# pasensio97/SDslam

Hardware: AMD Instinct MI355X
Metric: tracked frames/sec (ORB+ImageAlign+PnP) at 640x480, 1000 kp (higher is better)
Workload: dtype u8; 1 GPU; BASELINE configs[3] at the configs[1] pyramid: 640x480, 8-level x1.2, 1000 kp; ORB extract + ImageAlign (levels 4,3,2) + SearchByProjection + PnP RANSAC (maxIts 200; iterations actually run: tracking.mean_pnp_iterations with --full); pose_solver=pnp, pyramid=8x1.2, unique_scenes=64, inputs=resident in HBM, pose_records=packed on the device every step (single GPU: no collective)

## Files before the change

sdslam_amd/csrc/orb.hip:

```cpp
#include <hip/hip_runtime.h>

#include <algorithm>
#include <cstring>
#include <mutex>
#include <string>
#include <vector>

#include "introselect.h"
#include "introselect_wave.h"
#include "orb_plan.h"
#include "sd_common.h"
#include "sd_sincosf.h"

namespace sd {

static thread_local std::string g_err;
void set_error(const std::string& msg) { g_err = msg; }

#ifndef SD_XCD_REMAP
#define SD_XCD_REMAP 1
#endif
__device__ __forceinline__ void xcd_frame_block(unsigned& frame, unsigned& blk) {
#if SD_XCD_REMAP
  const unsigned nx = gridDim.x, total = nx * gridDim.y;
// ... 365 lines not shown
  for (int k = 0; k < 16; k++) {
    int m9 = min(min(m4[k], m4[(k + 4) & 15]), d[(k + 8) & 15]);
    int M9 = max(max(M4[k], M4[(k + 4) & 15]), d[(k + 8) & 15]);
    a = max(a, m9);
    b = min(b, M9);
  }
  return max(a, -b) - 1;
}

typedef unsigned short fu16;
__device__ __forceinline__ fu16 fmin16(fu16 a, fu16 b) { return a < b ? a : b; }
__device__ __forceinline__ fu16 fmax16(fu16 a, fu16 b) { return a > b ? a : b; }

typedef _Float16 fh2 __attribute__((ext_vector_type(2)));
typedef unsigned short fu2 __attribute__((ext_vector_type(2)));
__device__ __forceinline__ fh2 hmax3(fh2 a, fh2 b, fh2 c) { return __builtin_elementwise_maximum(__builtin_elementwise_maximum(a, b), c); }
__device__ __forceinline__ fh2 hmin3(fh2 a, fh2 b, fh2 c) { return __builtin_elementwise_minimum(__builtin_elementwise_minimum(a, b), c); }
__device__ __forceinline__ fh2 ring_pair(const uint8_t* __restrict__ ca, const uint8_t* __restrict__ cb, int o) {
  const fu2 r = {ca[o], cb[o]};
  return __builtin_bit_cast(fh2, r);
}
__device__ __forceinline__ void fast_ring_score2(const uint8_t* __restrict__ ca, const uint8_t* __restrict__ cb, int tp, int& sa, int& sb) {
  fh2 p[16];
  const int va = ca[0], vb = cb[0];
  p[0] = ring_pair(ca, cb, 3 * tp); p[1] = ring_pair(ca, cb, 3 * tp + 1); p[2] = ring_pair(ca, cb, 2 * tp + 2); p[3] = ring_pair(ca, cb, tp + 3);
  p[4] = ring_pair(ca, cb, 3); p[5] = ring_pair(ca, cb, -tp + 3); p[6] = ring_pair(ca, cb, -2 * tp + 2); p[7] = ring_pair(ca, cb, -3 * tp + 1);
  p[8] = ring_pair(ca, cb, -3 * tp); p[9] = ring_pair(ca, cb, -3 * tp - 1); p[10] = ring_pair(ca, cb, -2 * tp - 2); p[11] = ring_pair(ca, cb, -tp - 3);
  p[12] = ring_pair(ca, cb, -3); p[13] = ring_pair(ca, cb, tp - 3); p[14] = ring_pair(ca, cb, 2 * tp - 2); p[15] = ring_pair(ca, cb, 3 * tp - 1);
  fh2 x3[16], n3[16];
#pragma unroll
  for (int k = 0; k < 16; k++) {
    x3[k] = hmax3(p[k], p[(k + 1) & 15], p[(k + 2) & 15]);
    n3[k] = hmin3(p[k], p[(k + 1) & 15], p[(k + 2) & 15]);
  }
  fh2 x9[16], n9[16];
#pragma unroll
  for (int k = 0; k < 16; k++) {
    x9[k] = hmax3(x3[k], x3[(k + 3) & 15], x3[(k + 6) & 15]);
    n9[k] = hmin3(n3[k], n3[(k + 3) & 15], n3[(k + 6) & 15]);
  }
  fh2 A = hmin3(x9[0], x9[1], x9[2]), B = hmax3(n9[0], n9[1], n9[2]);
#pragma unroll
  for (int k = 3; k < 15; k += 2) {
    A = hmin3(A, x9[k], x9[k + 1]);
    B = hmax3(B, n9[k], n9[k + 1]);
  }
  A = __builtin_elementwise_minimum(A, x9[15]);
  B = __builtin_elementwise_maximum(B, n9[15]);
  const fu2 Au = __builtin_bit_cast(fu2, A), Bu = __builtin_bit_cast(fu2, B);
  sa = max(va - (int)Au.x, (int)Bu.x - va) - 1;
  sb = max(vb - (int)Au.y, (int)Bu.y - vb) - 1;
}

#ifdef SD_PNP_PROF
#define FPROF_FRAMES 256
#define FPROF_CELLS 192
__device__ unsigned long long g_fast_prof_wg[(size_t)FPROF_FRAMES * FPROF_CELLS * 8];
#define FPROF_DECL                                   \
  __shared__ unsigned long long s_fprof[8];          \
  if (threadIdx.x < 8) s_fprof[threadIdx.x] = 0;     \
  long long _pt = clock64()
#define FPROF(i)                                                                 \
  do {                                                                           \
    long long _n = clock64();                                                    \
    if (threadIdx.x == 0) s_fprof[i] += (unsigned long long)(_n - _pt);          \
    _pt = _n;                                                                    \
  } while (0)
#define FPROF_FLUSH                                                                                                   \
  do {                                                                                                                \
    if (threadIdx.x == 0 && frame < FPROF_FRAMES && cell < FPROF_CELLS)                                          \
      for (int _i = 0; _i < 8; _i++) g_fast_prof_wg[((size_t)frame * FPROF_CELLS + cell) * 8 + _i] = s_fprof[_i]; \
  } while (0)
#else
#define FPROF_DECL
#define FPROF(i)
#define FPROF_FLUSH
#endif

extern "C" __device__ __attribute__((const)) int __ockl_wfred_add_i32(int);

#ifndef FAST_STAGE_DEPTH
#define FAST_STAGE_DEPTH 12
#endif

struct FastSrc {
  uint32_t off[SD_MAX_LEVELS];
  int pstride[SD_MAX_LEVELS];
};

__global__ __launch_bounds__(256, 8) void k_fast_cells(const CellGeom* __restrict__ cells, const uint8_t* __restrict__ img0,
                                                    size_t frame_stride, const FastSrc src, int edge, uint32_t* __restrict__ cand,
                                                    uint32_t cand_per_frame, int32_t* __restrict__ cell_count, int ncells_total,
                                                    int cell0, int th) {
  extern __shared__ __attribute__((aligned(16))) uint8_t smem[];
  __shared__ int wcnt[4];
  unsigned uframe, ucell;
  xcd_frame_block(uframe, ucell);
  const int cell = (int)ucell + cell0;
  const CellGeom C = cells[cell];
  const int frame = (int)uframe;
  const int tid = threadIdx.x, lane = tid & 63;
  const int wave = __builtin_amdgcn_readfirstlane(tid >> 6);
  if (C.zw <= 0 || C.zh <= 0) {
    if (tid == 0) cell_count[(size_t)frame * ncells_total + cell] = 0;
    return;
  }
  const uint8_t* img = img0 + (size_t)frame * frame_stride + src.off[C.level];
  const int pstride = src.pstride[C.level];
  uint32_t* out = cand + (size_t)frame * cand_per_frame + C.cand_off;
  const int zw = C.zw, zh = C.zh, S = C.strip_rows;
  const int xs = C.zx0 - 3 + edge;
  const int xa = xs & ~3, sh = xs - xa;
  const int TPW = (sh + zw + 6 + 3) >> 2;
  const int TP = TPW * 4;
  const int SP = (zw + 2 + 3) & ~3;
  const int RPW = (S + 2 + 3) >> 2;
  const int QCAP = RPW * zw;
  uint8_t* tile = smem;
  uint8_t* sc = smem + (size_t)TP * (S + 2 + 6);
  uint16_t* queue = (uint16_t*)(sc + (size_t)SP * (S + 2 + 2)) + (size_t)wave * QCAP;
  const uint32_t qbase = (uint32_t)__builtin_amdgcn_readfirstlane((int)((size_t)TP * (S + 2 + 6) + (size_t)SP * (S + 2 + 2) + (size_t)wave * QCAP * 2));
  const unsigned magic = 0xFFFFFFFFu / (unsigned)zw + 1u;
  const unsigned magic_tpw = 0xFFFFFFFFu / (unsigned)TPW + 1u;
  const unsigned long long lt = lanemask_lt();
  int total = 0;
  FPROF_DECL;

  for (int r0 = 0; r0 < zh; r0 += S) {
    const int r1 = min(r0 + S, zh);
    const int sr0 = max(r0 - 1, 0), sr1 = min(r1 + 1, zh);
    const int nsr = sr1 - sr0;
    const int npr = nsr + 6;
    {
      const uint8_t* g = img + (size_t)(C.zy0 + sr0 - 3 + edge) * pstride + xa;
      const int ndw = __mul24(TPW, npr);
      int t0 = tid;
      asm volatile("" : "+v"(t0));
      for (int i0 = t0; i0 < ndw; i0 += 256 * FAST_STAGE_DEPTH) {
        uint32_t v[FAST_STAGE_DEPTH];
#pragma unroll
        for (int j = 0; j < FAST_STAGE_DEPTH; j++) {
          const int i = i0 + 256 * j;
          const int row = (int)__umulhi((unsigned)i, magic_tpw), wc = i - __mul24(row, TPW);
          v[j] = i < ndw ? *(const uint32_t*)(g + (uint32_t)(__mul24(row, pstride) + wc * 4)) : 0u;
        }
#pragma unroll
        for (int j = 0; j < FAST_STAGE_DEPTH; j++) {
          const int i = i0 + 256 * j;
          if (i < ndw) ((uint32_t*)tile)[i] = v[j];
        }
      }
      FPROF(7);
      const int nsc = ((nsr + 2) * SP) >> 2;
      for (int i = tid; i < nsc; i += 256) ((uint32_t*)sc)[i] = 0;
    }
    __syncthreads();
    FPROF(0);
    const int rpw = (nsr + 3) >> 2;
    const int y_lo = min(wave * rpw, nsr), y_hi = min(y_lo + rpw, nsr);
    int qn = 0;
    {
      const int i_lo = __mul24(y_lo, zw), i_hi = __mul24(y_hi, zw);
      const int pad = TP - zw;
      const uint8_t* tile0 = tile + 3 * TP + 3 + sh;
#ifdef FAST_SKIP_A
      for (int i0 = i_hi; i0 < i_hi; i0 += 64) {
#else
      for (int i0 = i_lo; i0 < i_hi; i0 += 64) {
#endif
        const int i = min(i0 + lane, i_hi - 1);
        const int y = (int)__umulhi((unsigned)i, magic);
        const uint8_t* c = tile0 + (i + __mul24(y, pad));
        const fu16 v = c[0], p0 = c[3 * TP], p4 = c[3], p8 = c[-3 * TP], p12 = c[-3];
        const fu16 D = fmax16(fmin16(p0, p8), fmin16(p4, p12));
        const fu16 Bt = fmin16(fmax16(p0, p8), fmax16(p4, p12));
        const short da = (short)(v - D), db = (short)(Bt - v);
        bool pass = (da > db ? da : db) > (short)th;
        if (i_hi - i0 < 64) pass = pass && (i0 + lane < i_hi);
        const unsigned long long m = __builtin_amdgcn_ballot_w64(pass);
        const int rank = (int)__builtin_amdgcn_mbcnt_hi((unsigned)(m >> 32), __builtin_amdgcn_mbcnt_lo((unsigned)m, 0u));
        if (pass) *(uint16_t*)(smem + (qbase + 2u * (uint32_t)(qn + rank))) = (uint16_t)i;
        qn += __popcll(m);
      }
    }
    FPROF(1);
#ifdef FAST_SKIP_B
    qn = 0;
#endif
    int cn = 0;
    for (int e0 = 0; e0 < qn; e0 += 128) {
      const int ea = e0 + lane, eb = ea + 64;
      bool corner_a = false, corner_b = false;
      unsigned qa = 0, qb = 0;
      if (ea < qn) {
        const bool has_b = eb < qn;
        qa = queue[ea];
        qb = has_b ? queue[eb] : qa;
        const int y_a = (int)__umulhi(qa, magic), x_a = (int)qa - __mul24(y_a, zw);
        const int y_b = (int)__umulhi(qb, magic), x_b = (int)qb - __mul24(y_b, zw);
        int sa, sb;
        fast_ring_score2(tile + __mul24(y_a + 3, TP) + x_a + 3 + sh, tile + __mul24(y_b + 3, TP) + x_b + 3 + sh, TP, sa, sb);
        corner_a = sa >= th;
        corner_b = has_b && sb >= th;
        if (corner_a && sa > 0) sc[__mul24(y_a + 1, SP) + x_a + 1] = (uint8_t)sa;
        if (corner_b && sb > 0) sc[__mul24(y_b + 1, SP) + x_b + 1] = (uint8_t)sb;
      }
      const unsigned long long ma = __builtin_amdgcn_ballot_w64(corner_a);
      if (corner_a) queue[cn + __popcll(ma & lt)] = (uint16_t)qa;
      cn += __popcll(ma);
      const unsigned long long mb = __builtin_amdgcn_ballot_w64(corner_b);
      if (corner_b) queue[cn + __popcll(mb & lt)] = (uint16_t)qb;
      cn += __popcll(mb);
    }
    qn = cn;
#ifdef FAST_SKIP_C
    qn = 0;
#endif
    FPROF(2);
    FPROF(3);
    __syncthreads();
    FPROF(4);
    {
      unsigned long long bits = 0;
      int cnt = 0;
      const int nj = (qn + 63) >> 6;
      for (int j = 0; j < nj; j++) {
        const int e = j * 64 + lane;
        bool keep = false;
        if (e < qn) {
          const unsigned q = queue[e];
          const int y = (int)__umulhi(q, magic), x = (int)q - __mul24(y, zw);
          const int yz = sr0 + y;
          const uint8_t* p = sc + __mul24(y + 1, SP) + x + 1;
          const int s = p[0];
          const int n0 = p[-1], n1 = p[1], n2 = p[-SP - 1], n3 = p[-SP], n4 = p[-SP + 1], n5 = p[SP - 1], n6 = p[SP], n7 = p[SP + 1];
          const int nm = max(max(max(n0, n1), n2), max(max(max(n3, n4), n5), max(n6, n7)));
          keep = (s > 0) & (s > nm) & (yz >= r0) & (yz < r1);
        }
        const unsigned long long m = __builtin_amdgcn_ballot_w64(keep);
        cnt += __popcll(m);
        bits |= (unsigned long long)keep << j;
      }
      if (lane == 0) wcnt[wave] = cnt;
      __syncthreads();
      int base = total;
      for (int w = 0; w < wave; w++) base += wcnt[w];
      const int strip_total = wcnt[0] + wcnt[1] + wcnt[2] + wcnt[3];
      for (int j = 0; j < nj; j++) {
        const bool keep = (bits >> j) & 1ull;
        const unsigned long long m = __builtin_amdgcn_ballot_w64(keep);
        if (keep) {
          const unsigned q = queue[j * 64 + lane];
          const int y = (int)__umulhi(q, magic), x = (int)q - __mul24(y, zw);
          const int s = sc[__mul24(y + 1, SP) + x + 1];
          const unsigned pos = (unsigned)(base + __popcll(m & lt));
          if (pos < C.cap)
            out[pos] = ((uint32_t)s << 24) | ((uint32_t)(C.zy0 + sr0 + y) << 12) | (uint32_t)(C.zx0 + x);
        }
        base += __popcll(m);
      }
      total += strip_total;
    }
    FPROF(5);
    __syncthreads();
    FPROF(6);
  }
  if (tid == 0) cell_count[(size_t)frame * ncells_total + cell] = min(total, (int)C.cap);
  FPROF_FLUSH;
}

#define SEL_WAVES 8
#define SEL_LIST_CAP 1536
#define SEL_MAX_CELLS 512
typedef __attribute__((address_space(3))) uint32_t lds_u32;

__global__ __launch_bounds__(64) void k_select_quota(const OrbPlan* __restrict__ P, const CellGeom* __restrict__ cells,
                                                     const int32_t* __restrict__ cell_count, int32_t* __restrict__ cell_keep,
                                                     int32_t* __restrict__ cell_off, int32_t* __restrict__ lvl_m) {
  extern __shared__ __attribute__((aligned(16))) int s_q[];
  const int frame = blockIdx.x, lane = threadIdx.x, nc = P->ncells;
  int* s_total = s_q;
  int* s_flag = s_q + nc;
  int* s_retain = s_q + 2 * nc;
  int* s_offv = s_q + 3 * nc;
  const int32_t* cc = cell_count + (size_t)frame * nc;
  for (int c = lane; c < nc; c += 64) {
    s_total[c] = cc[c];
    s_flag[c] = cells[c].evaluated;
  }
  sdsel::wave_fence();
  if (lane < P->nlevels) {
    const LevelGeom& L = P->lv[lane];
    int M = 0;
    if (L.ncells > 0 && L.quota > 0) {
      const int nC = L.ncells, c0 = L.cell0, nfc = L.nfeaturesCell;
      int nNoMore = 0, nToDistribute = 0;
      for (int c = c0; c < c0 + nC; c++) {
        const int nKeys = s_total[c];
        if (!s_flag[c]) {
          s_retain[c] = 0;
          s_flag[c] = 0;
          continue;
        }
        if (nKeys > nfc) {
          s_retain[c] = nfc;
          s_flag[c] = 0;
        } else {
          s_retain[c] = nKeys;
          nToDistribute += nfc - nKeys;
          s_flag[c] = 1;
          nNoMore++;
        }
      }
      while (nToDistribute > 0 && nNoMore < nC) {
        const int nNew = nfc + (int)ceilf((float)nToDistribute / (float)(nC - nNoMore));
        nToDistribute = 0;
        for (int c = c0; c < c0 + nC; c++) {
          if (!s_flag[c]) {
            if (s_total[c] > nNew) {
              s_retain[c] = nNew;
            } else {
              s_retain[c] = s_total[c];
              nToDistribute += nNew - s_total[c];
              s_flag[c] = 1;
              nNoMore++;
            }
          }
        }
      }
      for (int c = c0; c < c0 + nC; c++) {
        const int k = min(s_total[c], s_retain[c]);
        s_retain[c] = k;
        s_offv[c] = M;
        M += k;
      }
    } else {
      for (int c = L.cell0; c < L.cell0 + max(L.ncells, 0); c++) { s_retain[c] = 0; s_offv[c] = 0; }
// ... 455 lines not shown

static int build_geometry(sd_orb* h, const HostPlan& hp) {
  const size_t B = h->max_batch;
  const size_t slack = 4096;
  SD_HIP_CHECK(hipMalloc(&h->d_cells, std::max<size_t>(hp.cells.size(), 1) * sizeof(CellGeom)));
  SD_HIP_CHECK(hipMalloc(&h->d_tiles, std::max<size_t>(hp.blur_tiles.size(), 1) * sizeof(BlurTile)));
  SD_HIP_CHECK(hipMalloc(&h->d_coef, std::max<size_t>(hp.coef.size(), 1) * sizeof(int32_t)));
  for (int i = 0; i < h->nsets; i++) {
    SD_HIP_CHECK(hipMalloc(&h->pyr_set[i], hp.plan.pyr_frame_bytes * B + slack));
    SD_HIP_CHECK(hipMemsetAsync(h->pyr_set[i], 0, hp.plan.pyr_frame_bytes * B + slack, h->stream));
  }
  select_set(h, 0);
  SD_HIP_CHECK(hipMalloc(&h->d_blur, hp.plan.pyr_frame_bytes * B + slack));
  SD_HIP_CHECK(hipMalloc(&h->d_cand, std::max<size_t>(hp.plan.cand_per_frame, 1) * B * 4));
  SD_HIP_CHECK(hipMalloc(&h->d_scratch, std::max<size_t>(hp.plan.cand_per_frame, 1) * B * 4));
  SD_HIP_CHECK(hipMalloc(&h->d_cell_count, std::max<size_t>(hp.plan.ncells, 1) * B * 4));
  SD_HIP_CHECK(hipMalloc(&h->d_sel, std::max<size_t>(hp.plan.nsel, 1) * B * 4));
  SD_HIP_CHECK(hipMalloc(&h->d_sel_count, (size_t)h->nlevels * B * 4));
  SD_HIP_CHECK(hipMalloc(&h->d_cell_keep, std::max<size_t>(hp.plan.ncells, 1) * B * 4));
  SD_HIP_CHECK(hipMalloc(&h->d_cell_off, std::max<size_t>(hp.plan.ncells, 1) * B * 4));
  SD_HIP_CHECK(hipMalloc(&h->d_lvl_m, (size_t)h->nlevels * B * 4));
  SD_HIP_CHECK(hipMemsetAsync(h->d_blur, 0, hp.plan.pyr_frame_bytes * B + slack, h->stream));
  if (!hp.cells.empty())
    SD_HIP_CHECK(hipMemcpyAsync(h->d_cells, hp.cells.data(), hp.cells.size() * sizeof(CellGeom), hipMemcpyHostToDevice, h->stream));
  if (!hp.blur_tiles.empty())
    SD_HIP_CHECK(hipMemcpyAsync(h->d_tiles, hp.blur_tiles.data(), hp.blur_tiles.size() * sizeof(BlurTile), hipMemcpyHostToDevice, h->stream));
  if (!hp.coef.empty())
    SD_HIP_CHECK(hipMemcpyAsync(h->d_coef, hp.coef.data(), hp.coef.size() * sizeof(int32_t), hipMemcpyHostToDevice, h->stream));
  SD_HIP_CHECK(hipMemcpyAsync(h->d_plan, &hp.plan, sizeof(OrbPlan), hipMemcpyHostToDevice, h->stream));
  SD_HIP_CHECK(hipStreamSynchronize(h->stream));
  return SD_OK;
}

static int ensure_geometry(sd_orb* h, int w, int hgt) {
  if (h->have_geom && h->cur_w == w && h->cur_h == hgt) return SD_OK;
  SD_REQUIRE(w <= h->max_w && hgt <= h->max_h, SD_ERR_CAPACITY, "frame larger than the handle's max_w x max_h");
  const char* why = "";
  HostPlan np = h->hp;
  if (!plan_geometry(h->nfeatures, h->nlevels, h->thFAST, w, hgt, np, &why)) {
    set_error(std::string("unsupported geometry: ") + why);
    return SD_ERR_INVALID_ARG;
  }
  SD_REQUIRE(np.max_cells_per_level <= SEL_MAX_CELLS && (size_t)np.plan.ncells * 16 <= 60 * 1024, SD_ERR_INVALID_ARG,
             "too many grid cells (k_select_quota keeps four ints per cell in LDS)");
  SD_HIP_CHECK(hipSetDevice(h->device));
  SD_HIP_CHECK(hipStreamSynchronize(h->stream));
  { int rcw = wait_trackers(h); if (rcw != SD_OK) return rcw; }
  drop_graphs(h);
  h->select_recorded = false;
  h->have_geom = false;
  h->cur_w = h->cur_h = 0;
  h->last_frames = 0;
  free_geom(h);
  const int rc = build_geometry(h, np);
  if (rc != SD_OK) {
    free_geom(h);
    return rc;
  }
  h->hp = std::move(np);
  h->have_geom = true;
  h->cur_w = w;
  h->cur_h = hgt;
  return SD_OK;
}

static int pipeline_body(sd_orb* h, const uint8_t* d_imgs, int n, int stride, size_t frame_stride, bool prof, hipEvent_t* ev,
                         bool frames_ready, bool capturing) {
  const HostPlan& hp = h->hp;
  const OrbPlan& P = hp.plan;
  hipStream_t s = h->stream;
  bool fast_started = false;
  const bool fast_early = frames_ready && !capturing && h->select_recorded && h->stream == h->own_stream && opt(OPT_FAST0_EARLY) != 0;
  if (fast_early) SD_HIP_CHECK(hipStreamWaitEvent(h->fast_stream, h->ev_select_done, 0));
  SD_HIP_CHECK(hipEventRecord(h->ev_body_start, s));
  if (!fast_early) SD_HIP_CHECK(hipStreamWaitEvent(h->fast_stream, h->ev_body_start, 0));
  const bool pyr_early = fast_early && h->nsets == 2 && opt(OPT_PYR_EARLY) != 0;
  hipStream_t ps = pyr_early ? h->aux_stream : s;
  if (prof && !pyr_early) SD_HIP_CHECK(hipEventRecord(ev[0], s));
  if (pyr_early) {
    SD_HIP_CHECK(hipStreamWaitEvent(ps, h->ev_select_done, 0));
    if (prof) SD_HIP_CHECK(hipEventRecord(ev[0], ps));
  }
  const bool src_aligned = (((uintptr_t)d_imgs | (uintptr_t)stride | (uintptr_t)frame_stride) & 3) == 0;
  const bool fast0_direct = src_aligned && P.lv[0].ncells > 0 && opt(OPT_FAST0_FROM_FRAMES) != 0;
  const int ring_slot = h->ev_calls % sd_orb::kRing;
  int nfp = 0;
  auto fast_pair = [&](bool begin) {
    if (prof && h->evf_ready && nfp < sd_orb::kFastPairs) (void)hipEventRecord(h->evf[ring_slot][2 * nfp + (begin ? 0 : 1)], h->fast_stream);
    if (!begin) nfp++;
  };
  if (fast0_direct) {
    if (prof) SD_HIP_CHECK(hipEventRecord(ev[8], h->fast_stream));
    fast_started = true;
    FastSrc fs0;
    memset(&fs0, 0, sizeof(fs0));
    fs0.pstride[0] = stride;
    fast_pair(true);
    hipLaunchKernelGGL(k_fast_cells, dim3(P.lv[0].ncells, n), dim3(256), hp.fast_lds_level[0], h->fast_stream, h->d_cells, d_imgs,
                       frame_stride, fs0, 0, h->d_cand, P.cand_per_frame, h->d_cell_count, P.ncells, P.lv[0].cell0, P.thFAST);
    fast_pair(false);
  }
  FastSrc fsrc;
  memset(&fsrc, 0, sizeof(fsrc));
  for (int l = 0; l < P.nlevels; l++) {
    fsrc.off[l] = P.lv[l].off;
    fsrc.pstride[l] = P.lv[l].pstride;
  }
  const int merge_from = hp.fast_merge_from;
  for (int l = 0; l < P.nlevels; l++) {
    const LevelGeom& L = P.lv[l];
    const LevelGeom& S = P.lv[l > 0 ? l - 1 : 0];
    const bool split = L.w >= 16 && L.fast_resize != 0 && (l > 0 || src_aligned);
    if (!split) {
      dim3 grid((L.pstride + 255) / 256, (L.prows + 4 * PYR_ROWS - 1) / (4 * PYR_ROWS), n), block(64, 4, 1);
      hipLaunchKernelGGL(k_pyr_level, grid, block, 0, ps, L, S, (size_t)P.pyr_frame_bytes, l, d_imgs, stride, frame_stride, h->d_pyr);
    } else {
    auto magic = [](unsigned d) { return (unsigned)(0xFFFFFFFFull / d) + 1u; };
    const int G = (L.w + 2 * SD_EDGE + 3) / 4;
    const bool mirror = L.h >= 48;
    const int Hh = ((mirror ? L.h : L.prows) + PYR_RPT - 1) / PYR_RPT;
    const unsigned n_resize = (unsigned)(((size_t)Hh * G + 255) / 256);
    hipLaunchKernelGGL(k_pyr_split, dim3(n_resize, n), dim3(256), 0, ps, L, S, (size_t)P.pyr_frame_bytes, l, h->d_coef, d_imgs,
                       stride, frame_stride, h->d_pyr, G, magic((unsigned)G), Hh, mirror ? 1 : 0);
    }
    const bool merged = l >= merge_from;
    int ncl = L.ncells;
    size_t lds = hp.fast_lds_level[l];
    if (merged) {
      if (l != P.nlevels - 1) continue;
      ncl = 0;
      lds = 0;
      for (int m = merge_from; m < P.nlevels; m++) {
        ncl += P.lv[m].ncells;
        lds = std::max(lds, hp.fast_lds_level[m]);
      }
    }
    const int first = merged ? merge_from : l;
    if (ncl > 0 && !(l == 0 && fast0_direct)) {
      SD_HIP_CHECK(hipEventRecord(h->ev_level[l], ps));
      SD_HIP_CHECK(hipStreamWaitEvent(h->fast_stream, h->ev_level[l], 0));
      if (prof && !fast_started) SD_HIP_CHECK(hipEventRecord(ev[8], h->fast_stream));
      fast_started = true;
      fast_pair(true);
      hipLaunchKernelGGL(k_fast_cells, dim3(ncl, n), dim3(256), lds, h->fast_stream, h->d_cells, (const uint8_t*)h->d_pyr,
                         (size_t)P.pyr_frame_bytes, fsrc, SD_EDGE, h->d_cand, P.cand_per_frame, h->d_cell_count, P.ncells, P.lv[first].cell0,
                         P.thFAST);
      fast_pair(false);
    }
  }
  if (prof) SD_HIP_CHECK(hipEventRecord(ev[1], ps));
  SD_HIP_CHECK(hipEventRecord(h->ev_pyr_done, ps));
  SD_HIP_CHECK(hipStreamWaitEvent(h->aux_stream, h->ev_pyr_done, 0));
  if (pyr_early) SD_HIP_CHECK(hipStreamWaitEvent(h->aux_stream, h->ev_body_start, 0));
  if (prof) SD_HIP_CHECK(hipEventRecord(ev[3], h->aux_stream));
  hipLaunchKernelGGL(k_blur, dim3((unsigned)hp.blur_tiles.size(), n), dim3(256), 0, h->aux_stream, h->d_plan, h->d_tiles, h->d_pyr,
                     h->d_blur, h->d_sel_count);
  if (prof) SD_HIP_CHECK(hipEventRecord(ev[6], h->aux_stream));
  SD_HIP_CHECK(hipEventRecord(h->ev_blur_done, h->aux_stream));
  if (prof) {
    if (!fast_started) SD_HIP_CHECK(hipEventRecord(ev[8], h->fast_stream));
    SD_HIP_CHECK(hipEventRecord(ev[2], h->fast_stream));
    h->evf_n[ring_slot] = h->evf_ready ? nfp : 0;
  }
  SD_HIP_CHECK(hipStreamWaitEvent(h->fast_stream, h->ev_pyr_done, 0));
  SD_HIP_CHECK(hipEventRecord(h->ev_fast_done, h->fast_stream));
  SD_HIP_CHECK(hipStreamWaitEvent(s, h->ev_fast_done, 0));
  if (prof) SD_HIP_CHECK(hipEventRecord(ev[9], s));
  const int sel_cap = hp.max_cell_pixels > 12000 ? 1024 : 512;
  if (P.ncells > 0) {
    hipLaunchKernelGGL(k_select_quota, dim3(n), dim3(64), (size_t)P.ncells * 16, s, h->d_plan, h->d_cells, h->d_cell_count, h->d_cell_keep,
                       h->d_cell_off, h->d_lvl_m);
    int small_cap = 2 * sel_cap, big_cap = SEL_WAVES * sel_cap;
    if (const int e = opt(OPT_SELECT_SMALL_CAP)) small_cap = std::max(1, std::min(e, small_cap));
    if (const int e = opt(OPT_SELECT_BIG_CAP)) big_cap = std::max(small_cap, std::min(e, big_cap));
    hipLaunchKernelGGL(k_select_cells, dim3(P.ncells, n), dim3(64), (size_t)small_cap * 4 + 2 * WAVE_SEL_CAP * 2, s, h->d_plan, h->d_cells,
                       h->d_cand, h->d_cell_count, h->d_cell_keep, h->d_cell_off, h->d_scratch, small_cap);
    hipLaunchKernelGGL(k_select_bigcells, dim3(P.nlevels, n), dim3(64), (size_t)big_cap * 4 + 2 * WAVE_SEL_CAP * 2, s, h->d_plan, h->d_cells,
                       h->d_cand, h->d_cell_count, h->d_cell_keep, h->d_cell_off, h->d_scratch, small_cap, big_cap);
  }
  hipLaunchKernelGGL(k_select_final, dim3(P.nlevels, n), dim3(64), 0, s, h->d_plan, h->d_lvl_m, h->d_scratch, h->d_sel, h->d_sel_count);
  if (!capturing) {
    SD_HIP_CHECK(hipEventRecord(h->ev_select_done, s));
    h->select_recorded = true;
  }
  if (prof) SD_HIP_CHECK(hipEventRecord(ev[7], s));
  SD_HIP_CHECK(hipStreamWaitEvent(s, h->ev_blur_done, 0));
  if (prof) SD_HIP_CHECK(hipEventRecord(ev[4], s));
  const int cap = std::max(P.nsel, 1);
  {
    const int bpf = (cap + 4 * DESC_KPW - 1) / (4 * DESC_KPW);
    hipLaunchKernelGGL(k_orient_desc, dim3((unsigned)(((n + 7) / 8) * 8 * bpf)), dim3(256), 0, s, h->d_plan, h->d_pyr, h->d_blur,
                       h->d_sel, h->d_sel_count, h->d_kps, h->d_desc, h->d_nout, cap, n, bpf);
  }
  if (h->have_dist) {
    DistParams D;
    D.fx = h->dist_K[0]; D.fy = h->dist_K[1]; D.cx = h->dist_K[2]; D.cy = h->dist_K[3];
    for (int i = 0; i < 12; i++) D.k[i] = i < 5 ? (double)h->dist[i] : 0.0;
    hipLaunchKernelGGL(k_undistort, dim3((cap + 255) / 256, n), dim3(256), 0, s, h->d_kps, h->d_kps_un, h->d_nout, cap, D);
  }
  if (prof) SD_HIP_CHECK(hipEventRecord(ev[5], s));
  SD_HIP_CHECK(hipGetLastError());
  return SD_OK;
}

static void drop_graphs(sd_orb* h) {
  for (auto& g : h->graphs) {
    if (g.exec) (void)hipGraphExecDestroy(g.exec);
    g = sd_orb::GraphEntry();
  }
}

static int launch_pipeline(sd_orb* h, const uint8_t* d_imgs, int n, int stride, size_t frame_stride, bool frames_ready) {
  hipStream_t s = h->stream;
  const bool prof = h->profiling;
  hipEvent_t* ev = h->ev[h->ev_calls % sd_orb::kRing];
  select_set(h, (h->set + 1) % h->nsets);
  if (h->set_busy[h->set]) {
    SD_HIP_CHECK(hipStreamWaitEvent(s, h->ev_set_free[h->set], 0));
    if (h->nsets == 2) SD_HIP_CHECK(hipStreamWaitEvent(h->aux_stream, h->ev_set_free[h->set], 0));
    h->set_busy[h->set] = false;
  }
  const bool use_graph = opt(OPT_USE_GRAPH) != 0;
  int rc = SD_OK;
  if (prof || !use_graph) {
    rc = pipeline_body(h, d_imgs, n, stride, frame_stride, prof, ev, frames_ready, false);
  } else {
    sd_orb::GraphEntry* ge = nullptr;
    float dv[9] = {h->dist_K[0], h->dist_K[1], h->dist_K[2], h->dist_K[3], h->dist[0], h->dist[1], h->dist[2], h->dist[3], h->dist[4]};
    for (auto& g : h->graphs)
// ... 545 lines not shown
```

sdslam_amd/csrc/orb_plan.cpp:

```cpp
#include "orb_plan.h"
#include "sd_common.h"

#include <algorithm>
#include <cfloat>
#include <cmath>
#include <cstdlib>
#include <cstring>

namespace sd {

static inline int cv_round(float v) { return (int)lrintf(v); }
static inline int cv_round(double v) { return (int)lrint(v); }
static inline int cv_floor(double v) { int i = (int)v; return i - (i > v); }
static inline size_t up(size_t v, size_t a) { return (v + a - 1) / a * a; }

void plan_tables(int nfeatures, float scaleFactorArg, int nlevels, HostPlan& hp) {
  const double scaleFactor = scaleFactorArg;
  hp.sf.assign(nlevels, 1.0f);
  hp.sigma2.assign(nlevels, 1.0f);
  for (int i = 1; i < nlevels; i++) {
    hp.sf[i] = (float)(hp.sf[i - 1] * scaleFactor);
    hp.sigma2[i] = hp.sf[i] * hp.sf[i];
  }
  hp.inv_sf.resize(nlevels);
// ... 141 lines not shown
        L.cx = (int)hp.coef.size();
        hp.coef.insert(hp.coef.end(), xo.begin(), xo.end());
        hp.coef.insert(hp.coef.end(), xa.begin(), xa.end());
        L.cy = (int)hp.coef.size();
        hp.coef.insert(hp.coef.end(), yo.begin(), yo.end());
        hp.coef.insert(hp.coef.end(), yb.begin(), yb.end());
        bool ok = L.w >= 8;
        for (int x0 = 0; ok && x0 + 3 < L.w; x0++)
          if (std::min(xo[x0 + 3] + 1, S.w - 1) - xo[x0] > 7 || xo[x0 + 3] < xo[x0]) ok = false;
        for (int x = 0; ok && x < L.w; x++)
          if ((xa[x] & 0xffff) > 2048 || ((uint32_t)xa[x] >> 16) > 2048) ok = false;
        for (int y = 0; ok && y < L.h; y++)
          if (yo[y] < 0 || (yb[y] & 0xffff) > 2048 || ((uint32_t)yb[y] >> 16) > 2048) ok = false;
        L.fast_resize = ok ? 1 : 0;
        if (ok) ok = group_table(L, S.w, &xo, &xa, hp.coef);
        if (ok) {
          while (hp.coef.size() % 4) hp.coef.push_back(0);
          L.cr = (int)hp.coef.size();
          for (int y = 0; y < L.h; y++) {
            const int sy0 = std::min(yo[y], S.h - 1), sy1 = std::min(yo[y] + 1, S.h - 1);
            hp.coef.push_back((sy0 + SD_EDGE) * S.pstride + SD_EDGE);
            hp.coef.push_back((sy1 + SD_EDGE) * S.pstride + SD_EDGE);
            hp.coef.push_back(yb[y]);
            hp.coef.push_back(0);
          }
        }
        L.fast_resize = ok ? 1 : 0;
      }
    } else {
      L.fast_resize = group_table(L, 0, nullptr, nullptr, hp.coef) ? 1 : 0;
    }

    const int nDesired = L.quota;
    const int levelCols = (int)sqrtf((float)nDesired / (5 * imageRatio));
    const int levelRows = (int)(imageRatio * levelCols);
    L.cell0 = (int)hp.cells.size();
    L.cand_off = cand;
    L.cols = L.rows = L.ncells = 0;
    L.cellW = L.cellH = L.nfeaturesCell = 0;
    if (levelCols > 0 && levelRows > 0 && nDesired > 0) {
      const int minBX = SD_EDGE, minBY = SD_EDGE, maxBX = L.w - SD_EDGE, maxBY = L.h - SD_EDGE;
      const int W = maxBX - minBX, H = maxBY - minBY;
      const int cellW = (int)ceilf((float)W / levelCols);
      const int cellH = (int)ceilf((float)H / levelRows);
      L.cols = levelCols;
      L.rows = levelRows;
      L.cellW = cellW;
      L.cellH = cellH;
      L.ncells = levelCols * levelRows;
      L.nfeaturesCell = (int)ceilf((float)nDesired / L.ncells);
      for (int i = 0; i < levelRows; i++) {
        const int iniY = minBY + i * cellH - 3;
        int hY = cellH + 6;
        if (i == levelRows - 1) hY = maxBY + 3 - iniY;
        for (int j = 0; j < levelCols; j++) {
          const int iniX = minBX + j * cellW - 3;
          int hX = cellW + 6;
          if (j == levelCols - 1) hX = maxBX + 3 - iniX;
          CellGeom c;
          c.level = l;
          bool skip = (i == levelRows - 1 && hY <= 0) || (j == levelCols - 1 && hX <= 0) || iniX < 0 ||
                      iniY < 0 || hX < 0 || hY < 0 || iniX + hX > L.w || iniY + hY > L.h;
          bool ok = !skip && hX > 6 && hY > 6;
          c.evaluated = skip ? 0 : 1;
          c.zx0 = iniX + 3;
          c.zy0 = iniY + 3;
          c.zw = ok ? hX - 6 : 0;
          c.zh = ok ? hY - 6 : 0;
          if (c.zw == 1) { *why = "a grid cell's FAST zone is one pixel wide (frame too small for this many features per level)"; return false; }
          c.cap = ok ? (uint32_t)(((c.zw + 1) / 2) * ((c.zh + 1) / 2)) : 0;
          c.cand_off = cand;
          cand += c.cap;
          c.strip_rows = 0;
          if (ok) hp.max_cell_pixels = std::max(hp.max_cell_pixels, c.zw * c.zh);
          if (ok) {
            const size_t lds_kb = (size_t)opt(OPT_FAST_LDS_KB);
            const size_t whole_kb = (size_t)opt(OPT_FAST_LDS_WHOLE_KB);
            int S = c.zh;
            bool whole_pass = l < hp.fast_merge_from;
            if (!whole_pass) S = std::min(c.zh, std::max(1, 12288 / c.zw));
            for (;;) {
              size_t tp = up((size_t)c.zw + 6 + 3, 4), sp = up((size_t)c.zw + 2, 4);
              size_t rpw = (size_t)(S + 2 + 3) / 4;
              size_t need = tp * (S + 2 + 6) + sp * (S + 2 + 2) + 2 * 4 * rpw * c.zw + 64;
              const size_t budget = whole_pass ? std::max(whole_kb, lds_kb) : lds_kb;
              bool fits = need <= budget * 1024 && rpw * c.zw <= 4096 && (size_t)(S + 2) * c.zw < 65536;
              if (whole_pass && !fits) {
                whole_pass = false;
                S = std::min(c.zh, std::max(1, 12288 / c.zw));
                continue;
              }
              if (fits || S == 1) {
                lds_max = std::max(lds_max, need);
                hp.fast_lds_level[l] = std::max(hp.fast_lds_level[l], need);
                break;
              }
              S = std::max(1, S - std::max(1, S / 8));
            }
            c.strip_rows = S;
          }
          hp.cells.push_back(c);
        }
      }
    }
    L.cand_cap = cand - L.cand_off;
    hp.max_cells_per_level = std::max(hp.max_cells_per_level, L.ncells);

    {
      const int nstrips = (L.w + 63) / 64, npairs = nstrips * ((L.h + 31) / 32);
      for (int p0 = 0; p0 < npairs; p0 += 16)
        hp.blur_tiles.push_back(BlurTile{l, p0, nstrips, (unsigned)(0xFFFFFFFFull / (unsigned)nstrips) + 1u});
    }
  }
  P.ncells = (int)hp.cells.size();
  P.nsel = sel;
  P.cand_per_frame = cand;
  P.pyr_frame_bytes = off;
  hp.fast_lds_bytes = lds_max;
  if (hp.coef.empty()) hp.coef.push_back(0);

  hp.stage_bytes[0] = (sum_px - px_last) + (sum_px - px0) + px0 * 2;
  hp.stage_bytes[1] = sum_px;
  hp.stage_bytes[2] = (double)cand * 0 + (double)sel * 4;
  hp.stage_bytes[3] = 2 * sum_px;
  hp.stage_bytes[4] = (double)sel * (749 + 961 + 28 + 32);
  return true;
}

}
```

Before: 235,400 frames/s.

## Stage FAST tiles with 16-byte loads and store tile offsets in candidate queue

Aligns the FAST tile staging to 16-byte boundaries and loads global pixels with 128-bit vector loads when the source is 16-byte aligned, cutting the number of load instructions. The score map now shares the tile pitch, so the candidate queue stores tile offsets directly instead of packed cell indices. This drops the per-candidate divide/multiply index recomputation in the scoring and NMS stages. It costs somewhat larger LDS footprints from the 16-byte pitch padding, which the planner now accounts for, possibly lowering occupancy.

```diff
diff --git a/sdslam_amd/csrc/orb.hip b/sdslam_amd/csrc/orb.hip
--- a/sdslam_amd/csrc/orb.hip
+++ b/sdslam_amd/csrc/orb.hip
@@ -471,6 +471,7 @@
 #ifndef FAST_STAGE_DEPTH
 #define FAST_STAGE_DEPTH 12
 #endif
+typedef uint32_t fast_u4 __attribute__((ext_vector_type(4)));
 
 struct FastSrc {
   uint32_t off[SD_MAX_LEVELS];
@@ -480,7 +481,7 @@
 __global__ __launch_bounds__(256, 8) void k_fast_cells(const CellGeom* __restrict__ cells, const uint8_t* __restrict__ img0,
                                                     size_t frame_stride, const FastSrc src, int edge, uint32_t* __restrict__ cand,
                                                     uint32_t cand_per_frame, int32_t* __restrict__ cell_count, int ncells_total,
-                                                    int cell0, int th) {
+                                                    int cell0, int th, int wide16) {
   extern __shared__ __attribute__((aligned(16))) uint8_t smem[];
   __shared__ int wcnt[4];
   unsigned uframe, ucell;
@@ -499,18 +500,20 @@
   uint32_t* out = cand + (size_t)frame * cand_per_frame + C.cand_off;
   const int zw = C.zw, zh = C.zh, S = C.strip_rows;
   const int xs = C.zx0 - 3 + edge;
-  const int xa = xs & ~3, sh = xs - xa;
-  const int TPW = (sh + zw + 6 + 3) >> 2;
-  const int TP = TPW * 4;
-  const int SP = (zw + 2 + 3) & ~3;
-  const int RPW = (S + 2 + 3) >> 2;
+  const int xa = xs & ~15, sh = xs - xa;
+  const int TPU = (sh + zw + 6 + 15) >> 4;
+  const int TP = TPU * 16;
+  const int NSR = min(S + 2, zh);
+  const int RPW = (NSR + 3) >> 2;
   const int QCAP = RPW * zw;
   uint8_t* tile = smem;
-  uint8_t* sc = smem + (size_t)TP * (S + 2 + 6);
-  uint16_t* queue = (uint16_t*)(sc + (size_t)SP * (S + 2 + 2)) + (size_t)wave * QCAP;
-  const uint32_t qbase = (uint32_t)__builtin_amdgcn_readfirstlane((int)((size_t)TP * (S + 2 + 6) + (size_t)SP * (S + 2 + 2) + (size_t)wave * QCAP * 2));
+  uint8_t* sc = smem + (size_t)TP * (NSR + 6);
+  uint16_t* queue = (uint16_t*)(sc + (size_t)TP * (NSR + 2)) + (size_t)wave * QCAP;
+  const uint32_t qbase = (uint32_t)__builtin_amdgcn_readfirstlane((int)((size_t)TP * (2 * NSR + 8) + (size_t)wave * QCAP * 2));
   const unsigned magic = 0xFFFFFFFFu / (unsigned)zw + 1u;
-  const unsigned magic_tpw = 0xFFFFFFFFu / (unsigned)TPW + 1u;
+  const unsigned magic_tp = 0xFFFFFFFFu / (unsigned)TP + 1u;
+  const uint8_t* tile0 = tile + 3 * TP + 3 + sh;
+  uint8_t* sc0 = sc + TP + 1;
   const unsigned long long lt = lanemask_lt();
   int total = 0;
   FPROF_DECL;
@@ -522,26 +525,47 @@
     const int npr = nsr + 6;
     {
       const uint8_t* g = img + (size_t)(C.zy0 + sr0 - 3 + edge) * pstride + xa;
-      const int ndw = __mul24(TPW, npr);
       int t0 = tid;
       asm volatile("" : "+v"(t0));
-      for (int i0 = t0; i0 < ndw; i0 += 256 * FAST_STAGE_DEPTH) {
-        uint32_t v[FAST_STAGE_DEPTH];
-#pragma unroll
-        for (int j = 0; j < FAST_STAGE_DEPTH; j++) {
-          const int i = i0 + 256 * j;
-          const int row = (int)__umulhi((unsigned)i, magic_tpw), wc = i - __mul24(row, TPW);
-          v[j] = i < ndw ? *(const uint32_t*)(g + (uint32_t)(__mul24(row, pstride) + wc * 4)) : 0u;
+      if (wide16) {
+        const int nu = __mul24(TPU, npr);
+        const unsigned magic_tpu = 0x80000000u / (unsigned)TPU;
+        for (int i0 = t0; i0 < nu; i0 += 256 * (FAST_STAGE_DEPTH / 4)) {
+          fast_u4 v[FAST_STAGE_DEPTH / 4];
+#pragma unroll
+          for (int j = 0; j < FAST_STAGE_DEPTH / 4; j++) {
+            const int i = i0 + 256 * j;
+            const int row = (int)__umulhi(2u * (unsigned)i + 1u, magic_tpu), uc = i - __mul24(row, TPU);
+            v[j] = i < nu ? *(const fast_u4*)(g + (uint32_t)(__mul24(row, pstride) + uc * 16)) : fast_u4{0u, 0u, 0u, 0u};
+          }
+#pragma unroll
+          for (int j = 0; j < FAST_STAGE_DEPTH / 4; j++) {
+            const int i = i0 + 256 * j;
+            if (i < nu) ((fast_u4*)tile)[i] = v[j];
+          }
         }
-#pragma unroll
-        for (int j = 0; j < FAST_STAGE_DEPTH; j++) {
-          const int i = i0 + 256 * j;
-          if (i < ndw) ((uint32_t*)tile)[i] = v[j];
+      } else {
+        const int TPW = TPU * 4;
+        const int ndw = __mul24(TPW, npr);
+        const unsigned magic_tpw = 0xFFFFFFFFu / (unsigned)TPW + 1u;
+        for (int i0 = t0; i0 < ndw; i0 += 256 * FAST_STAGE_DEPTH) {
+          uint32_t v[FAST_STAGE_DEPTH];
+#pragma unroll
+          for (int j = 0; j < FAST_STAGE_DEPTH; j++) {
+            const int i = i0 + 256 * j;
+            const int row = (int)__umulhi((unsigned)i, magic_tpw), wc = i - __mul24(row, TPW);
+            v[j] = i < ndw ? *(const uint32_t*)(g + (uint32_t)(__mul24(row, pstride) + wc * 4)) : 0u;
+          }
+#pragma unroll
+          for (int j = 0; j < FAST_STAGE_DEPTH; j++) {
+            const int i = i0 + 256 * j;
+            if (i < ndw) ((uint32_t*)tile)[i] = v[j];
+          }
         }
       }
       FPROF(7);
-      const int nsc = ((nsr + 2) * SP) >> 2;
-      for (int i = tid; i < nsc; i += 256) ((uint32_t*)sc)[i] = 0;
+      const int nsc = __mul24(nsr + 2, TPU);
+      for (int i = tid; i < nsc; i += 256) ((fast_u4*)sc)[i] = fast_u4{0u, 0u, 0u, 0u};
     }
     __syncthreads();
     FPROF(0);
@@ -551,7 +575,6 @@
     {
       const int i_lo = __mul24(y_lo, zw), i_hi = __mul24(y_hi, zw);
       const int pad = TP - zw;
-      const uint8_t* tile0 = tile + 3 * TP + 3 + sh;
 #ifdef FAST_SKIP_A
       for (int i0 = i_hi; i0 < i_hi; i0 += 64) {
 #else
@@ -559,7 +582,8 @@
 #endif
         const int i = min(i0 + lane, i_hi - 1);
         const int y = (int)__umulhi((unsigned)i, magic);
-        const uint8_t* c = tile0 + (i + __mul24(y, pad));
+        const int ofs = i + __mul24(y, pad);
+        const uint8_t* c = tile0 + ofs;
         const fu16 v = c[0], p0 = c[3 * TP], p4 = c[3], p8 = c[-3 * TP], p12 = c[-3];
         const fu16 D = fmax16(fmin16(p0, p8), fmin16(p4, p12));
         const fu16 Bt = fmin16(fmax16(p0, p8), fmax16(p4, p12));
@@ -568,7 +592,7 @@
         if (i_hi - i0 < 64) pass = pass && (i0 + lane < i_hi);
         const unsigned long long m = __builtin_amdgcn_ballot_w64(pass);
         const int rank = (int)__builtin_amdgcn_mbcnt_hi((unsigned)(m >> 32), __builtin_amdgcn_mbcnt_lo((unsigned)m, 0u));
-        if (pass) *(uint16_t*)(smem + (qbase + 2u * (uint32_t)(qn + rank))) = (uint16_t)i;
+        if (pass) *(uint16_t*)(smem + (qbase + 2u * (uint32_t)(qn + rank))) = (uint16_t)ofs;
         qn += __popcll(m);
       }
     }
@@ -585,14 +609,12 @@
         const bool has_b = eb < qn;
         qa = queue[ea];
         qb = has_b ? queue[eb] : qa;
-        const int y_a = (int)__umulhi(qa, magic), x_a = (int)qa - __mul24(y_a, zw);
-        const int y_b = (int)__umulhi(qb, magic), x_b = (int)qb - __mul24(y_b, zw);
         int sa, sb;
-        fast_ring_score2(tile + __mul24(y_a + 3, TP) + x_a + 3 + sh, tile + __mul24(y_b + 3, TP) + x_b + 3 + sh, TP, sa, sb);
+        fast_ring_score2(tile0 + qa, tile0 + qb, TP, sa, sb);
         corner_a = sa >= th;
         corner_b = has_b && sb >= th;
-        if (corner_a && sa > 0) sc[__mul24(y_a + 1, SP) + x_a + 1] = (uint8_t)sa;
-        if (corner_b && sb > 0) sc[__mul24(y_b + 1, SP) + x_b + 1] = (uint8_t)sb;
+        if (corner_a && sa > 0) sc0[qa] = (uint8_t)sa;
+        if (corner_b && sb > 0) sc0[qb] = (uint8_t)sb;
       }
       const unsigned long long ma = __builtin_amdgcn_ballot_w64(corner_a);
       if (corner_a) queue[cn + __popcll(ma & lt)] = (uint16_t)qa;
@@ -613,18 +635,17 @@
       unsigned long long bits = 0;
       int cnt = 0;
       const int nj = (qn + 63) >> 6;
+      const unsigned own_lo = (unsigned)__mul24(r0 - sr0, TP), own_n = (unsigned)__mul24(r1 - r0, TP);
       for (int j = 0; j < nj; j++) {
         const int e = j * 64 + lane;
         bool keep = false;
         if (e < qn) {
           const unsigned q = queue[e];
-          const int y = (int)__umulhi(q, magic), x = (int)q - __mul24(y, zw);
-          const int yz = sr0 + y;
-          const uint8_t* p = sc + __mul24(y + 1, SP) + x + 1;
+          const uint8_t* p = sc0 + q;
           const int s = p[0];
-          const int n0 = p[-1], n1 = p[1], n2 = p[-SP - 1], n3 = p[-SP], n4 = p[-SP + 1], n5 = p[SP - 1], n6 = p[SP], n7 = p[SP + 1];
+          const int n0 = p[-1], n1 = p[1], n2 = p[-TP - 1], n3 = p[-TP], n4 = p[-TP + 1], n5 = p[TP - 1], n6 = p[TP], n7 = p[TP + 1];
           const int nm = max(max(max(n0, n1), n2), max(max(max(n3, n4), n5), max(n6, n7)));
-          keep = (s > 0) & (s > nm) & (yz >= r0) & (yz < r1);
+          keep = (s > 0) & (s > nm) & (q - own_lo < own_n);
         }
         const unsigned long long m = __builtin_amdgcn_ballot_w64(keep);
         cnt += __popcll(m);
@@ -640,8 +661,8 @@
         const unsigned long long m = __builtin_amdgcn_ballot_w64(keep);
         if (keep) {
           const unsigned q = queue[j * 64 + lane];
-          const int y = (int)__umulhi(q, magic), x = (int)q - __mul24(y, zw);
-          const int s = sc[__mul24(y + 1, SP) + x + 1];
+          const int y = (int)__umulhi(q, magic_tp), x = (int)q - __mul24(y, TP);
+          const int s = sc0[q];
           const unsigned pos = (unsigned)(base + __popcll(m & lt));
           if (pos < C.cap)
             out[pos] = ((uint32_t)s << 24) | ((uint32_t)(C.zy0 + sr0 + y) << 12) | (uint32_t)(C.zx0 + x);
@@ -1263,6 +1284,7 @@
     if (prof) SD_HIP_CHECK(hipEventRecord(ev[0], ps));
   }
   const bool src_aligned = (((uintptr_t)d_imgs | (uintptr_t)stride | (uintptr_t)frame_stride) & 3) == 0;
+  const bool src_wide = (((uintptr_t)d_imgs | (uintptr_t)stride | (uintptr_t)frame_stride) & 15) == 0;
   const bool fast0_direct = src_aligned && P.lv[0].ncells > 0 && opt(OPT_FAST0_FROM_FRAMES) != 0;
   const int ring_slot = h->ev_calls % sd_orb::kRing;
   int nfp = 0;
@@ -1278,7 +1300,7 @@
     fs0.pstride[0] = stride;
     fast_pair(true);
     hipLaunchKernelGGL(k_fast_cells, dim3(P.lv[0].ncells, n), dim3(256), hp.fast_lds_level[0], h->fast_stream, h->d_cells, d_imgs,
-                       frame_stride, fs0, 0, h->d_cand, P.cand_per_frame, h->d_cell_count, P.ncells, P.lv[0].cell0, P.thFAST);
+                       frame_stride, fs0, 0, h->d_cand, P.cand_per_frame, h->d_cell_count, P.ncells, P.lv[0].cell0, P.thFAST, src_wide ? 1 : 0);
     fast_pair(false);
   }
   FastSrc fsrc;
@@ -1325,7 +1347,7 @@
       fast_pair(true);
       hipLaunchKernelGGL(k_fast_cells, dim3(ncl, n), dim3(256), lds, h->fast_stream, h->d_cells, (const uint8_t*)h->d_pyr,
                          (size_t)P.pyr_frame_bytes, fsrc, SD_EDGE, h->d_cand, P.cand_per_frame, h->d_cell_count, P.ncells, P.lv[first].cell0,
-                         P.thFAST);
+                         P.thFAST, 1);
       fast_pair(false);
     }
   }
diff --git a/sdslam_amd/csrc/orb_plan.cpp b/sdslam_amd/csrc/orb_plan.cpp
--- a/sdslam_amd/csrc/orb_plan.cpp
+++ b/sdslam_amd/csrc/orb_plan.cpp
@@ -247,9 +247,13 @@
             for (;;) {
               size_t tp = up((size_t)c.zw + 6 + 3, 4), sp = up((size_t)c.zw + 2, 4);
               size_t rpw = (size_t)(S + 2 + 3) / 4;
+              const size_t tp16 = up((size_t)c.zw + 6 + 15, 16);
               size_t need = tp * (S + 2 + 6) + sp * (S + 2 + 2) + 2 * 4 * rpw * c.zw + 64;
               const size_t budget = whole_pass ? std::max(whole_kb, lds_kb) : lds_kb;
-              bool fits = need <= budget * 1024 && rpw * c.zw <= 4096 && (size_t)(S + 2) * c.zw < 65536;
+              bool fits = need <= budget * 1024 && rpw * c.zw <= 4096 && (size_t)(std::min(S + 2, c.zh) + 1) * tp16 <= 65536;
+              const size_t nsr = (size_t)std::min(S + 2, c.zh);
+              need = tp16 * (nsr + 6) + tp16 * (nsr + 2) + 2 * 4 * ((nsr + 3) / 4) * c.zw + 64;
+              fits = fits && need <= std::max(budget * 1024, (size_t)65536);
               if (whole_pass && !fits) {
                 whole_pass = false;
                 S = std::min(c.zh, std::max(1, 12288 / c.zw));
```

New measurement: 237,800 frames/s (median of 6 runs). 1.0% higher.
